# NUS-HPC-AI-Lab/VideoSys

Measured on AMD Instinct MI355X. Metric: videos/min (Open-Sora 512x512x64f, 30 denoise steps, DiT denoising only) + sec/denoise-step, higher is better.
Workload: dtype bf16; 1 GPU; open-sora-v1.2 STDiT3-XL/2 512x512x64f, latent [4,19,64,64], CFG batch 2 = 38912 token rows, 300 text tokens, depth 28; steps_per_video=30, parallelism=dsp1

## Files before the change

videosys_amd/csrc/rowwise.hip:

```cpp
#include "common.h"

#include <cstdlib>
#include "vsys_internal.h"

namespace vsys {
namespace {

template <int MAXV>
__global__ __launch_bounds__(256) void adaln_modulate_kernel(const bf16_t* __restrict__ x, const bf16_t* __restrict__ shift,
                                                             const bf16_t* __restrict__ scale, bf16_t* __restrict__ y,
                                                             int64_t rows, int C, int64_t rows_per_sample,
                                                             int64_t mod_stride, float eps) {
  const int lane = threadIdx.x & 63;
  const int64_t row = (int64_t)blockIdx.x * 4 + (threadIdx.x >> 6);
  if (row >= rows) return;
  const int nchunk = C >> 3;
  const bf16_t* xr = x + row * C;
  float v[MAXV][8];
  float s = 0.f;
#pragma unroll
  for (int i = 0; i < MAXV; ++i) {
    const int c = lane + 64 * i;
    if (c < nchunk) {
      uint4 u = *reinterpret_cast<const uint4*>(xr + c * 8);
// ... 184 lines not shown
    unpack8(*reinterpret_cast<const uint4*>(gate + b * gate_stride + alt + c * 8), g);
#pragma unroll
    for (int k = 0; k < 8; ++k) a[k] += bf2f(f2bf(g[k] * v[k]));
    reinterpret_cast<uint4*>(x)[i] = pack8(a);
  }
}

__global__ void im2col_patch_kernel(const float* __restrict__ z, int Bz, bf16_t* __restrict__ out, int B, int F, int Cin, int H,
                                    int W, int p) {
  const int Hp = H / p, Wp = W / p, K = Cin * p * p;
  const int64_t total = (int64_t)B * F * Hp * Wp * K;
  for (int64_t i = (int64_t)blockIdx.x * blockDim.x + threadIdx.x; i < total; i += (int64_t)gridDim.x * blockDim.x) {
    const int k = (int)(i % K);
    const int64_t tok = i / K;
    const int wp = (int)(tok % Wp), hp = (int)((tok / Wp) % Hp), f = (int)((tok / ((int64_t)Wp * Hp)) % F);
    const int b = (int)(tok / ((int64_t)Wp * Hp * F));
    const int dx = k % p, dy = (k / p) % p, c = k / (p * p);
    out[i] = f2bf(z[((((int64_t)(b % Bz) * F + f) * Cin + c) * H + hp * p + dy) * W + wp * p + dx]);
  }
}

__global__ void unpatchify_cvx_kernel(const bf16_t* __restrict__ x, int64_t ldx, float* __restrict__ out, int B, int F, int Hp,
                                      int Wp, int Cout, int p) {
  const int H = Hp * p, W = Wp * p;
  const int64_t total = (int64_t)B * F * Cout * H * W;
  for (int64_t i = (int64_t)blockIdx.x * blockDim.x + threadIdx.x; i < total; i += (int64_t)gridDim.x * blockDim.x) {
    const int w = (int)(i % W), h = (int)((i / W) % H), c = (int)((i / ((int64_t)W * H)) % Cout);
    const int64_t bf = i / ((int64_t)W * H * Cout);
    const int64_t tok = (bf * Hp + h / p) * Wp + w / p;
    out[i] = bf2f(x[tok * ldx + (c * p + h % p) * p + w % p]);
  }
}

__global__ void mod_table_kernel(const bf16_t* __restrict__ table, const bf16_t* __restrict__ t_mlp, bf16_t* __restrict__ out,
                                 int nblk, int B, int C6) {
  const int64_t i = (int64_t)blockIdx.x * blockDim.x + threadIdx.x;
  const int64_t total = (int64_t)nblk * B * C6;
  if (i >= total) return;
  const int c = (int)(i % C6);
  const int b = (int)((i / C6) % B);
  const int k = (int)(i / ((int64_t)C6 * B));
  out[i] = f2bf(bf2f(table[(int64_t)k * C6 + c]) + bf2f(t_mlp[(int64_t)b * C6 + c]));
}

__global__ void timestep_embedding_kernel(const float* __restrict__ t, bf16_t* __restrict__ out, int B, int dim) {
  const int i = blockIdx.x * blockDim.x + threadIdx.x;
  const int half = dim / 2;
  if (i >= B * half) return;
  const int b = i / half, k = i - b * half;
  const float f = expf(-9.210340371976184f * (float)k / (float)half);
  const float a = t[b] * f;
  out[(int64_t)b * dim + k] = f2bf(cosf(a));
  out[(int64_t)b * dim + half + k] = f2bf(sinf(a));
}

__global__ __launch_bounds__(256) void patch_embed_kernel(const float* __restrict__ x, int Bz, const bf16_t* __restrict__ w,
                                                          const bf16_t* __restrict__ bias, const bf16_t* __restrict__ pos,
                                                          bf16_t* __restrict__ out, int B, int Cin, int T, int H, int W,
                                                          int ph, int pw, int C, int s0, int Sl) {
  const int Hp = (H + ph - 1) / ph, Wp = (W + pw - 1) / pw;
  const int S = Hp * Wp;
  const int cchunks = C >> 3;
  const int64_t total = (int64_t)B * T * Sl * cchunks;
  const int64_t i = (int64_t)blockIdx.x * blockDim.x + threadIdx.x;
  if (i >= total) return;
  const int cc = (int)(i % cchunks);
  const int64_t tok = i / cchunks;
  const int s = s0 + (int)(tok % Sl);
  const int t = (int)((tok / Sl) % T);
  const int b = (int)(tok / ((int64_t)Sl * T));
  const int bz = b % Bz;
  if (s >= S) {
    *reinterpret_cast<uint4*>(out + tok * C + cc * 8) = make_uint4(0, 0, 0, 0);
    return;
  }
  const int hp = s / Wp, wp = s - hp * Wp;
  float acc[8];
  {
    float bb[8];
    unpack8(*reinterpret_cast<const uint4*>(bias + cc * 8), bb);
#pragma unroll
    for (int e = 0; e < 8; ++e) acc[e] = bb[e];
  }
  const int K = Cin * ph * pw;
  if (K == 16) {
    float xin[16];
#pragma unroll
    for (int k = 0; k < 16; ++k) {
      const int ci = k >> 2, dy = (k >> 1) & 1, dx = k & 1;
      const int hh = hp * 2 + dy, ww = wp * 2 + dx;
      xin[k] = 0.f;
      if (ph == 2 && pw == 2 && hh < H && ww < W) xin[k] = bf2f(f2bf(x[((((int64_t)bz * Cin + ci) * T + t) * H + hh) * W + ww]));
    }
    if (ph == 2 && pw == 2) {
#pragma unroll
      for (int e = 0; e < 8; ++e) {
        const bf16_t* wr = w + (int64_t)(cc * 8 + e) * 16;
        float wa[8], wb[8];
        unpack8(*reinterpret_cast<const uint4*>(wr), wa);
        unpack8(*reinterpret_cast<const uint4*>(wr + 8), wb);
#pragma unroll
        for (int k = 0; k < 8; ++k) acc[e] += xin[k] * wa[k] + xin[k + 8] * wb[k];
      }
    }
  }
  if (!(K == 16 && ph == 2 && pw == 2)) {
    for (int ci = 0; ci < Cin; ++ci)
      for (int dy = 0; dy < ph; ++dy)
        for (int dx = 0; dx < pw; ++dx) {
          const int hh = hp * ph + dy, ww = wp * pw + dx;
          float xv = 0.f;
          if (hh < H && ww < W) xv = bf2f(f2bf(x[((((int64_t)bz * Cin + ci) * T + t) * H + hh) * W + ww]));
          const int k = (ci * ph + dy) * pw + dx;
#pragma unroll
          for (int e = 0; e < 8; ++e) acc[e] += xv * bf2f(w[(int64_t)(cc * 8 + e) * K + k]);
        }
  }
  float pp[8];
  unpack8(*reinterpret_cast<const uint4*>(pos + (int64_t)s * C + cc * 8), pp);
#pragma unroll
  for (int e = 0; e < 8; ++e) acc[e] = bf2f(f2bf(acc[e])) + pp[e];
  *reinterpret_cast<uint4*>(out + tok * C + cc * 8) = pack8(acc);
}

template <int MAXV>
__global__ __launch_bounds__(256) void final_layer_kernel(const bf16_t* __restrict__ x, const bf16_t* __restrict__ table,
                                                          const bf16_t* __restrict__ tvec, const bf16_t* __restrict__ w,
                                                          const bf16_t* __restrict__ bias, float* __restrict__ out,
                                                          int B, int T, int Hp, int Wp, int H, int W, int ph, int pw,
                                                          int Cout, int C, float eps, int Sl, float* __restrict__ tokens) {
  const int lane = threadIdx.x & 63;
  const int S = Sl;
  const int64_t rows = (int64_t)B * T * S;
  const int64_t row = (int64_t)blockIdx.x * 4 + (threadIdx.x >> 6);
  if (row >= rows) return;
  const int nchunk = C >> 3;
  const bf16_t* xr = x + row * C;
  float v[MAXV][8];
  float s = 0.f;
#pragma unroll
  for (int i = 0; i < MAXV; ++i) {
    const int c = lane + 64 * i;
    if (c < nchunk) {
      unpack8(*reinterpret_cast<const uint4*>(xr + c * 8), v[i]);
#pragma unroll
      for (int e = 0; e < 8; ++e) s += v[i][e];
    } else {
#pragma unroll
      for (int e = 0; e < 8; ++e) v[i][e] = 0.f;
    }
  }
  const float mean = wave_sum(s) / (float)C;
  float q = 0.f;
#pragma unroll
  for (int i = 0; i < MAXV; ++i) {
    const int c = lane + 64 * i;
    if (c < nchunk) {
#pragma unroll
      for (int e = 0; e < 8; ++e) {
        float d = v[i][e] - mean;
        q += d * d;
      }
    }
  }
  const float rstd = rsqrtf(wave_sum(q) / (float)C + eps);
  const int b = (int)(row / ((int64_t)T * S));
#pragma unroll
  for (int i = 0; i < MAXV; ++i) {
    const int c = lane + 64 * i;
    if (c < nchunk) {
      float sh[8], sc[8], tt[8];
      unpack8(*reinterpret_cast<const uint4*>(table + c * 8), sh);
      unpack8(*reinterpret_cast<const uint4*>(table + C + c * 8), sc);
      unpack8(*reinterpret_cast<const uint4*>(tvec + (int64_t)b * C + c * 8), tt);
#pragma unroll
      for (int e = 0; e < 8; ++e) {
        const float shift = bf2f(f2bf(sh[e] + tt[e])), scale = bf2f(f2bf(sc[e] + tt[e]));
        v[i][e] = bf2f(f2bf((v[i][e] - mean) * rstd * (1.0f + scale) + shift));
      }
    }
  }
  const int NOUT = ph * pw * Cout;
  const int64_t tok = row % ((int64_t)T * S);
  const int t = (int)(tok / S), sidx = (int)(tok % S);
  const int hp = sidx / Wp, wp = sidx - hp * Wp;
  for (int n = 0; n < NOUT; ++n) {
    const bf16_t* wr = w + (int64_t)n * C;
    float d = 0.f;
#pragma unroll
    for (int i = 0; i < MAXV; ++i) {
      const int c = lane + 64 * i;
      if (c < nchunk) {
        float ww[8];
        unpack8(*reinterpret_cast<const uint4*>(wr + c * 8), ww);
#pragma unroll
        for (int e = 0; e < 8; ++e) d += v[i][e] * ww[e];
      }
    }
    d = wave_sum(d);
    if (lane == 0) {
      d = bf2f(f2bf(d + bf2f(bias[n])));
      if (tokens != nullptr) {
        tokens[row * NOUT + n] = d;
        continue;
      }
      const int co = n % Cout;
      const int dx = (n / Cout) % pw, dy = n / (Cout * pw);
      const int hh = hp * ph + dy, ww2 = wp * pw + dx;
      if (hh < H && ww2 < W) out[((((int64_t)b * Cout + co) * T + t) * H + hh) * W + ww2] = d;
    }
  }
}

__global__ void unpatchify_tokens_kernel(const float* __restrict__ tok, float* __restrict__ out, int P, int B, int T, int Sl,
                                         int Hp, int Wp, int H, int W, int ph, int pw, int Cout) {
  const int NOUT = ph * pw * Cout;
  const int64_t total = (int64_t)B * Cout * T * H * W;
  const int64_t i = (int64_t)blockIdx.x * blockDim.x + threadIdx.x;
  if (i >= total) return;
  const int ww = (int)(i % W), hh = (int)((i / W) % H), t = (int)((i / ((int64_t)W * H)) % T);
  const int co = (int)((i / ((int64_t)W * H * T)) % Cout), b = (int)(i / ((int64_t)W * H * T * Cout));
  const int hp = hh / ph, dy = hh - hp * ph, wp = ww / pw, dx = ww - wp * pw;
  const int s = hp * Wp + wp;
  const int r = s / Sl, j = s - r * Sl;
  const int n = (dy * pw + dx) * Cout + co;
  out[i] = tok[((((int64_t)r * B + b) * T + t) * Sl + j) * NOUT + n];
}

__global__ void cfg_euler_kernel(float* __restrict__ z, const float* __restrict__ model_out, int Bz, int Cin, int Cout,
                                 int64_t thw, float guidance, float dt) {
  const int64_t i = (int64_t)blockIdx.x * blockDim.x + threadIdx.x;
  const int64_t total = (int64_t)Bz * Cin * thw;
  if (i >= total) return;
  const int64_t sp = i % thw;
  const int c = (int)((i / thw) % Cin);
  const int b = (int)(i / (thw * Cin));
  const float cond = model_out[((int64_t)b * Cout + c) * thw + sp];
  const float unc = model_out[((int64_t)(b + Bz) * Cout + c) * thw + sp];
  z[i] = z[i] + (unc + guidance * (cond - unc)) * dt;
}

__global__ void cfg_axpby_kernel(float* __restrict__ z, const float* __restrict__ model_out, int Bz, int Cin, int Cout,
                                 int64_t thw, float guidance, float c_z, float c_eps, int cond_first) {
  const int64_t i = (int64_t)blockIdx.x * blockDim.x + threadIdx.x;
  const int64_t total = (int64_t)Bz * Cin * thw;
  if (i >= total) return;
  const int64_t sp = i % thw;
  const int c = (int)((i / thw) % Cin);
  const int b = (int)(i / (thw * Cin));
  const float h0 = model_out[((int64_t)b * Cout + c) * thw + sp];
  const float h1 = model_out[((int64_t)(b + Bz) * Cout + c) * thw + sp];
  const float cond = cond_first ? h0 : h1, unc = cond_first ? h1 : h0;
  z[i] = c_z * z[i] + c_eps * (unc + guidance * (cond - unc));
}

__global__ void add_bcast_rows_kernel(bf16_t* __restrict__ x, const bf16_t* __restrict__ e, int64_t rows, int C8, int64_t group,
                                      int64_t period) {
  const int64_t total = rows * C8;
  for (int64_t i = (int64_t)blockIdx.x * blockDim.x + threadIdx.x; i < total; i += (int64_t)gridDim.x * blockDim.x) {
    const int64_t r = i / C8;
    const int c = (int)(i - r * C8);
    const int64_t er = (r / group) % period;
    float a[8], b[8];
    unpack8(reinterpret_cast<const uint4*>(x)[i], a);
// ... 21 lines not shown
  for (int64_t i = (int64_t)blockIdx.x * blockDim.x + threadIdx.x; i < total; i += (int64_t)gridDim.x * blockDim.x) {
    const int64_t r = i / C8;
    const int c = (int)(i - r * C8) * 8;
    float x[8], y[8];
    unpack8(*reinterpret_cast<const uint4*>(a + r * lda + c), x);
    unpack8(*reinterpret_cast<const uint4*>(b + r * ldb + c), y);
#pragma unroll
    for (int e = 0; e < 8; ++e) x[e] = bf2f(f2bf(x[e] * scale)) + y[e];
    *reinterpret_cast<uint4*>(out + r * ldo + c) = pack8(x);
  }
}

__global__ void copy_4d_kernel(const bf16_t* __restrict__ src, bf16_t* __restrict__ dst, int n0, int n1, int n2, int C,
                               int64_t ss0, int64_t ss1, int64_t ss2, int64_t ds0, int64_t ds1, int64_t ds2,
                               int n1_valid, int n2_valid) {
  const int cch = C >> 3;
  const int64_t total = (int64_t)n0 * n1 * n2 * cch;
  for (int64_t i = (int64_t)blockIdx.x * blockDim.x + threadIdx.x; i < total; i += (int64_t)gridDim.x * blockDim.x) {
    const int c = (int)(i % cch);
    int64_t r = i / cch;
    const int i2 = (int)(r % n2);
    r /= n2;
    const int i1 = (int)(r % n1);
    const int i0 = (int)(r / n1);
    uint4 v = make_uint4(0, 0, 0, 0);
    if (i1 < n1_valid && i2 < n2_valid) v = *reinterpret_cast<const uint4*>(src + i0 * ss0 + i1 * ss1 + i2 * ss2 + c * 8);
    *reinterpret_cast<uint4*>(dst + i0 * ds0 + i1 * ds1 + i2 * ds2 + c * 8) = v;
  }
}

struct CopyBatch {
  int nops;
  CopyDesc d[VSYS_COPY_BATCH_MAX];
};
__global__ void copy_4d_batch_kernel(const bf16_t* __restrict__ src, bf16_t* __restrict__ dst, CopyBatch b) {
  const CopyDesc& o = b.d[blockIdx.y];
  const int cch = o.C >> 3;
  const int64_t total = (int64_t)o.n0 * o.n1 * o.n2 * cch;
  const bf16_t* s = src + o.src_off;
  bf16_t* d = dst + o.dst_off;
  for (int64_t i = (int64_t)blockIdx.x * blockDim.x + threadIdx.x; i < total; i += (int64_t)gridDim.x * blockDim.x) {
    const int c = (int)(i % cch);
    int64_t r = i / cch;
    const int i2 = (int)(r % o.n2);
    r /= o.n2;
    const int i1 = (int)(r % o.n1);
    const int i0 = (int)(r / o.n1);
    uint4 v = make_uint4(0, 0, 0, 0);
    if (i1 < o.n1_valid && i2 < o.n2_valid) v = *reinterpret_cast<const uint4*>(s + i0 * o.ss0 + i1 * o.ss1 + i2 * o.ss2 + c * 8);
    *reinterpret_cast<uint4*>(d + i0 * o.ds0 + i1 * o.ds1 + i2 * o.ds2 + c * 8) = v;
  }
}

}

int launch_copy_4d_batch(const bf16_t* src, bf16_t* dst, const CopyDesc* ops, int nops, hipStream_t stream) {
  if (nops <= 0) return 0;
  if (nops > VSYS_COPY_BATCH_MAX) return VSYS_ERR_SHAPE;
  CopyBatch b;
  b.nops = nops;
  int64_t most = 0;
  for (int i = 0; i < nops; ++i) {
    if (ops[i].C % 8 || ops[i].n0 < 0 || ops[i].n1 < 0 || ops[i].n2 < 0) return VSYS_ERR_SHAPE;
    b.d[i] = ops[i];
    const int64_t t = (int64_t)ops[i].n0 * ops[i].n1 * ops[i].n2 * (ops[i].C / 8);
    most = t > most ? t : most;
  }
  if (most <= 0) return 0;
  int64_t grid = (most + 255) / 256;
  if (grid > 2048) grid = 2048;
  hipLaunchKernelGGL(copy_4d_batch_kernel, dim3((unsigned)grid, (unsigned)nops), dim3(256), 0, stream, src, dst, b);
  return hipGetLastError() == hipSuccess ? 0 : VSYS_ERR_LAUNCH;
}

int launch_adaln_modulate(const bf16_t* x, const bf16_t* shift, const bf16_t* scale, bf16_t* y, int64_t rows, int C,
                          int64_t rows_per_sample, int64_t mod_stride, float eps, hipStream_t stream) {
  if (rows <= 0) return 0;
  if (C % 8 != 0 || C > 64 * 8 * 4 || rows_per_sample <= 0 || (mod_stride % 8)) return VSYS_ERR_SHAPE;
  if (C > 64 * 8 * 2 && C <= 64 * 8 * 3 && rows_per_sample % 2 == 0) {
    hipLaunchKernelGGL(adaln_modulate_rows_kernel<2>, dim3((unsigned)((rows + 7) / 8)), dim3(256), 0, stream, x, shift, scale, y, rows, C,
                       rows_per_sample, mod_stride, eps);
    return hipGetLastError() == hipSuccess ? 0 : VSYS_ERR_LAUNCH;
  }
  const unsigned grid = (unsigned)((rows + 3) / 4);
  if (C <= 64 * 8 * 2)
    hipLaunchKernelGGL(adaln_modulate_kernel<2>, dim3(grid), dim3(256), 0, stream, x, shift, scale, y, rows, C,
                       rows_per_sample, mod_stride, eps);
  else if (C <= 64 * 8 * 3)
    hipLaunchKernelGGL(adaln_modulate_kernel<3>, dim3(grid), dim3(256), 0, stream, x, shift, scale, y, rows, C,
                       rows_per_sample, mod_stride, eps);
  else
    hipLaunchKernelGGL(adaln_modulate_kernel<4>, dim3(grid), dim3(256), 0, stream, x, shift, scale, y, rows, C,
                       rows_per_sample, mod_stride, eps);
  return hipGetLastError() == hipSuccess ? 0 : VSYS_ERR_LAUNCH;
}

int launch_ln_modulate(const bf16_t* x, const bf16_t* ln_w, const bf16_t* ln_b, const bf16_t* shift, const bf16_t* scale,
                       bf16_t* y, int64_t rows, int C, int64_t rows_per_sample, int64_t mod_stride, int64_t seg_split,
                       int64_t mod_alt, float eps, hipStream_t stream) {
  if (rows <= 0) return 0;
  if (C % 8 != 0 || C > 64 * 8 * 6 || rows_per_sample <= 0 || (mod_stride % 8) || (mod_alt % 8)) return VSYS_ERR_SHAPE;
  if ((ln_w == nullptr) != (ln_b == nullptr) || (shift == nullptr) != (scale == nullptr)) return VSYS_ERR_ARG;
  const unsigned grid = (unsigned)((rows + 3) / 4);
#define VSYS_LNMOD(V)                                                                                                      \
  hipLaunchKernelGGL(ln_modulate_kernel<V>, dim3(grid), dim3(256), 0, stream, x, ln_w, ln_b, shift, scale, y, rows, C,       \
                     rows_per_sample, mod_stride, seg_split, mod_alt, eps)
// ... 10 lines not shown
  if (rows <= 0) return 0;
  if (C % 8 || rows_per_sample <= 0 || (gate_stride % 8) || (gate_alt % 8)) return VSYS_ERR_SHAPE;
  int64_t grid = (rows * (C / 8) + 255) / 256;
  if (grid > 2048 * 4) grid = 2048 * 4;
  hipLaunchKernelGGL(gate_add_rows_kernel, dim3((unsigned)grid), dim3(256), 0, stream, x, y, gate, rows, C / 8, rows_per_sample,
                     gate_stride, seg_split, gate_alt);
  return hipGetLastError() == hipSuccess ? 0 : VSYS_ERR_LAUNCH;
}

int launch_im2col_patch(const float* z, int Bz, bf16_t* out, int B, int F, int Cin, int H, int W, int p, hipStream_t stream) {
  if (p <= 0 || H % p || W % p || Bz <= 0) return VSYS_ERR_SHAPE;
  const int64_t total = (int64_t)B * F * (H / p) * (W / p) * Cin * p * p;
  if (total <= 0) return 0;
  int64_t grid = (total + 255) / 256;
  if (grid > 2048 * 8) grid = 2048 * 8;
  hipLaunchKernelGGL(im2col_patch_kernel, dim3((unsigned)grid), dim3(256), 0, stream, z, Bz, out, B, F, Cin, H, W, p);
  return hipGetLastError() == hipSuccess ? 0 : VSYS_ERR_LAUNCH;
}

int launch_unpatchify_cvx(const bf16_t* x, int64_t ldx, float* out, int B, int F, int Hp, int Wp, int Cout, int p,
                          hipStream_t stream) {
  const int64_t total = (int64_t)B * F * Cout * Hp * p * Wp * p;
  if (total <= 0) return 0;
  int64_t grid = (total + 255) / 256;
  if (grid > 2048 * 8) grid = 2048 * 8;
  hipLaunchKernelGGL(unpatchify_cvx_kernel, dim3((unsigned)grid), dim3(256), 0, stream, x, ldx, out, B, F, Hp, Wp, Cout, p);
  return hipGetLastError() == hipSuccess ? 0 : VSYS_ERR_LAUNCH;
}

int launch_mod_table(const bf16_t* table, const bf16_t* t_mlp, bf16_t* out, int nblk, int B, int C6, hipStream_t stream) {
  const int64_t total = (int64_t)nblk * B * C6;
  if (total <= 0) return 0;
  hipLaunchKernelGGL(mod_table_kernel, dim3((unsigned)((total + 255) / 256)), dim3(256), 0, stream, table, t_mlp, out, nblk,
                     B, C6);
  return hipGetLastError() == hipSuccess ? 0 : VSYS_ERR_LAUNCH;
}

int launch_timestep_embedding(const float* t, bf16_t* out, int B, int dim, hipStream_t stream) {
  if (dim % 2) return VSYS_ERR_SHAPE;
  const int total = B * (dim / 2);
  if (total <= 0) return 0;
  hipLaunchKernelGGL(timestep_embedding_kernel, dim3((total + 127) / 128), dim3(128), 0, stream, t, out, B, dim);
  return hipGetLastError() == hipSuccess ? 0 : VSYS_ERR_LAUNCH;
}

int launch_patch_embed(const float* x, int Bz, const bf16_t* w, const bf16_t* bias, const bf16_t* pos, bf16_t* out, int B,
                       int Cin, int T, int H, int W, int ph, int pw, int C, int s0, int Sl, hipStream_t stream) {
  if (C % 8 || Bz <= 0 || s0 < 0) return VSYS_ERR_SHAPE;
  const int Hp = (H + ph - 1) / ph, Wp = (W + pw - 1) / pw;
  if (Sl < 0) Sl = Hp * Wp;
  const int64_t total = (int64_t)B * T * Sl * (C / 8);
  if (total <= 0) return 0;
  if ((total + 255) / 256 > 0x7fffffff) return VSYS_ERR_SHAPE;
  hipLaunchKernelGGL(patch_embed_kernel, dim3((unsigned)((total + 255) / 256)), dim3(256), 0, stream, x, Bz, w, bias, pos, out,
                     B, Cin, T, H, W, ph, pw, C, s0, Sl);
  return hipGetLastError() == hipSuccess ? 0 : VSYS_ERR_LAUNCH;
}

int launch_unpatchify_tokens(const float* tok, float* out, int P, int B, int T, int Sl, int Hp, int Wp, int H, int W, int ph,
                             int pw, int Cout, hipStream_t stream) {
  if (P <= 0 || Sl <= 0 || (int64_t)P * Sl < (int64_t)Hp * Wp) return VSYS_ERR_SHAPE;
  const int64_t total = (int64_t)B * Cout * T * H * W;
  if (total <= 0) return 0;
  if ((total + 255) / 256 > 0x7fffffff) return VSYS_ERR_SHAPE;
  hipLaunchKernelGGL(unpatchify_tokens_kernel, dim3((unsigned)((total + 255) / 256)), dim3(256), 0, stream, tok, out, P, B, T, Sl,
                     Hp, Wp, H, W, ph, pw, Cout);
  return hipGetLastError() == hipSuccess ? 0 : VSYS_ERR_LAUNCH;
}

int launch_final_layer(const bf16_t* x, const bf16_t* table, const bf16_t* tvec, const bf16_t* w, const bf16_t* bias,
                       float* out, int B, int T, int Hp, int Wp, int H, int W, int ph, int pw, int Cout, int C, float eps,
                       int Sl, float* tokens, hipStream_t stream) {
  if (C % 8 != 0 || C > 64 * 8 * 4) return VSYS_ERR_SHAPE;
  if (Sl < 0) Sl = Hp * Wp;
  if (tokens == nullptr && Sl != Hp * Wp) return VSYS_ERR_ARG;
  const int64_t rows = (int64_t)B * T * Sl;
  if (rows <= 0) return 0;
  const unsigned grid = (unsigned)((rows + 3) / 4);
  if (C <= 64 * 8 * 2)
    hipLaunchKernelGGL(final_layer_kernel<2>, dim3(grid), dim3(256), 0, stream, x, table, tvec, w, bias, out, B, T, Hp, Wp,
                       H, W, ph, pw, Cout, C, eps, Sl, tokens);
  else if (C <= 64 * 8 * 3)
    hipLaunchKernelGGL(final_layer_kernel<3>, dim3(grid), dim3(256), 0, stream, x, table, tvec, w, bias, out, B, T, Hp, Wp,
                       H, W, ph, pw, Cout, C, eps, Sl, tokens);
  else
    hipLaunchKernelGGL(final_layer_kernel<4>, dim3(grid), dim3(256), 0, stream, x, table, tvec, w, bias, out, B, T, Hp, Wp,
                       H, W, ph, pw, Cout, C, eps, Sl, tokens);
  return hipGetLastError() == hipSuccess ? 0 : VSYS_ERR_LAUNCH;
}

int launch_cfg_euler(float* z, const float* model_out, int Bz, int Cin, int Cout, int64_t thw, float guidance, float dt,
                     hipStream_t stream) {
  const int64_t total = (int64_t)Bz * Cin * thw;
  if (total <= 0) return 0;
  hipLaunchKernelGGL(cfg_euler_kernel, dim3((unsigned)((total + 255) / 256)), dim3(256), 0, stream, z, model_out, Bz, Cin,
                     Cout, thw, guidance, dt);
  return hipGetLastError() == hipSuccess ? 0 : VSYS_ERR_LAUNCH;
}

int launch_cfg_axpby(float* z, const float* model_out, int Bz, int Cin, int Cout, int64_t thw, float guidance, float c_z,
                     float c_eps, int cond_first, hipStream_t stream) {
  const int64_t total = (int64_t)Bz * Cin * thw;
  if (total <= 0) return 0;
  hipLaunchKernelGGL(cfg_axpby_kernel, dim3((unsigned)((total + 255) / 256)), dim3(256), 0, stream, z, model_out, Bz, Cin,
                     Cout, thw, guidance, c_z, c_eps, cond_first);
  return hipGetLastError() == hipSuccess ? 0 : VSYS_ERR_LAUNCH;
}

int launch_add_bcast_rows(bf16_t* x, const bf16_t* e, int64_t rows, int C, int64_t group, int64_t period, hipStream_t stream) {
  if (rows <= 0) return 0;
  if (C % 8 || group <= 0 || period <= 0) return VSYS_ERR_SHAPE;
  int64_t grid = (rows * (C / 8) + 255) / 256;
  if (grid > 2048 * 4) grid = 2048 * 4;
  hipLaunchKernelGGL(add_bcast_rows_kernel, dim3((unsigned)grid), dim3(256), 0, stream, x, e, rows, C / 8, group, period);
  return hipGetLastError() == hipSuccess ? 0 : VSYS_ERR_LAUNCH;
}

int launch_add_rows(bf16_t* x, const bf16_t* y, int64_t n, hipStream_t stream) {
  if (n <= 0) return 0;
  if (n % 8) return VSYS_ERR_SHAPE;
  const int64_t n8 = n / 8;
  int64_t grid = (n8 + 255) / 256;
  if (grid > 2048 * 4) grid = 2048 * 4;
  hipLaunchKernelGGL(add_rows_kernel, dim3((unsigned)grid), dim3(256), 0, stream, x, y, n8);
  return hipGetLastError() == hipSuccess ? 0 : VSYS_ERR_LAUNCH;
}

int launch_scale_add_rows(const bf16_t* a, int64_t lda, const bf16_t* b, int64_t ldb, bf16_t* out, int64_t ldo, int64_t rows, int C,
                          float scale, hipStream_t stream) {
  if (rows < 0 || C < 0) return VSYS_ERR_SHAPE;
// ... 25 lines not shown
```

Baseline: 21.73 videos/min.

## Add LDS-staged final layer and register-tiled patch-embed kernels

Adds a specialized patch-embed kernel for 4-channel 2x2 patches. It keeps each thread's weight slice in registers, stages input patches in shared memory, prefetches positional embeddings, and writes the result once per CFG batch copy. Adds a final-layer kernel that stages the projection weights and modulation vectors in LDS, prefetches the next row, and reduces 16 outputs at once with butterfly shuffles instead of one wave reduction per output. Both kernels size their grids from the CU count and are selected by default unless an environment flag requests the reference path. These are small per-step kernels compared with the 28 transformer blocks, so their share of end-to-end time is limited.

```diff
diff --git a/videosys_amd/csrc/rowwise.hip b/videosys_amd/csrc/rowwise.hip
--- a/videosys_amd/csrc/rowwise.hip
+++ b/videosys_amd/csrc/rowwise.hip
@@ -418,6 +418,258 @@
       if (hh < H && ww2 < W) out[((((int64_t)b * Cout + co) * T + t) * H + hh) * W + ww2] = d;
     }
   }
+}
+
+
+constexpr int PE_TOKENS = 64;
+constexpr int PE_THREADS = 512;
+__global__ __launch_bounds__(PE_THREADS, 2) void patch_embed_k16_kernel(
+    const float* __restrict__ x, int Bz, const bf16_t* __restrict__ w, const bf16_t* __restrict__ bias,
+    const bf16_t* __restrict__ pos, bf16_t* __restrict__ out, int B, int T, int H, int W, int C, int s0, int Sl, int cpb, int tpb,
+    int ntok, int U) {
+  __shared__ __attribute__((aligned(16))) float xs[PE_TOKENS * 16];
+  constexpr int Cin = 4;
+  const int Hp = (H + 1) / 2, Wp = (W + 1) / 2;
+  const int S = Hp * Wp;
+  const int cchunks = C >> 3;
+  const int u0 = blockIdx.x * ntok;
+  const int u1 = U - u0 < ntok ? U : u0 + ntok;
+  const int slot = threadIdx.x / cpb;
+  const int cc = blockIdx.y * cpb + (threadIdx.x - slot * cpb);
+  const bool active = slot < tpb && cc < cchunks;
+  float wf[8][16], bb[8];
+  int j = 0, t = 0, bz = 0;
+  int ucur = u0 + slot;
+  uint4 upn = make_uint4(0, 0, 0, 0);
+  if (active) {
+#pragma unroll
+    for (int e = 0; e < 8; ++e) {
+      const bf16_t* wr = w + (int64_t)(cc * 8 + e) * 16;
+      unpack8(*reinterpret_cast<const uint4*>(wr), wf[e]);
+      unpack8(*reinterpret_cast<const uint4*>(wr + 8), wf[e] + 8);
+    }
+    unpack8(*reinterpret_cast<const uint4*>(bias + cc * 8), bb);
+    j = ucur % Sl;
+    t = (ucur / Sl) % T;
+    bz = ucur / Sl / T;
+    if (ucur < u1 && s0 + j < S) upn = *reinterpret_cast<const uint4*>(pos + (int64_t)(s0 + j) * C + cc * 8);
+  }
+  const int batch = PE_TOKENS / tpb * tpb;
+  for (int ub = u0; ub < u1; ub += batch) {
+    const int n = u1 - ub < batch ? u1 - ub : batch;
+    for (int idx = threadIdx.x; idx < n * 16; idx += blockDim.x) {
+      const int k = idx & 15;
+      const int u = ub + (idx >> 4);
+      const int s = s0 + u % Sl;
+      const int tt = (u / Sl) % T;
+      const int bb0 = u / Sl / T;
+      float xv = 0.f;
+      if (s < S) {
+        const int hp = s / Wp, wp = s - hp * Wp;
+        const int ci = k >> 2, dy = (k >> 1) & 1, dx = k & 1;
+        const int hh = hp * 2 + dy, ww = wp * 2 + dx;
+        if (hh < H && ww < W) xv = bf2f(f2bf(x[((((int64_t)bb0 * Cin + ci) * T + tt) * H + hh) * W + ww]));
+      }
+      xs[idx] = xv;
+    }
+    __syncthreads();
+    if (active) {
+      for (; ucur < ub + n; ucur += tpb) {
+        const int i = ucur - ub;
+        const int s = s0 + j;
+        const uint4 up = upn;
+        int jn = j + tpb, tn = t, bn = bz;
+        while (jn >= Sl) {
+          jn -= Sl;
+          if (++tn == T) {
+            tn = 0;
+            ++bn;
+          }
+        }
+        if (u1 - ucur > tpb && s0 + jn < S) upn = *reinterpret_cast<const uint4*>(pos + (int64_t)(s0 + jn) * C + cc * 8);
+        uint4 o = make_uint4(0, 0, 0, 0);
+        if (s < S) {
+          float xin[16];
+#pragma unroll
+          for (int q = 0; q < 4; ++q) {
+            const float4 f = *reinterpret_cast<const float4*>(xs + i * 16 + q * 4);
+            xin[q * 4 + 0] = f.x; xin[q * 4 + 1] = f.y; xin[q * 4 + 2] = f.z; xin[q * 4 + 3] = f.w;
+          }
+          float acc[8];
+#pragma unroll
+          for (int e = 0; e < 8; ++e) acc[e] = bb[e];
+#pragma unroll
+          for (int e = 0; e < 8; ++e) {
+            const float* wa = wf[e];
+            const float* wb = wf[e] + 8;
+#pragma unroll
+            for (int k = 0; k < 8; ++k) acc[e] += xin[k] * wa[k] + xin[k + 8] * wb[k];
+          }
+          float pp[8];
+          unpack8(up, pp);
+#pragma unroll
+          for (int e = 0; e < 8; ++e) acc[e] = bf2f(f2bf(acc[e])) + pp[e];
+          o = pack8(acc);
+        }
+        for (int b = bz; b < B; b += Bz) *reinterpret_cast<uint4*>(out + (((int64_t)b * T + t) * Sl + j) * C + cc * 8) = o;
+        j = jn;
+        t = tn;
+        bz = bn;
+      }
+    }
+    __syncthreads();
+  }
+}
+
+constexpr int FL_THREADS = 512;
+__device__ __forceinline__ void fmac(float& d, float a, float b) { asm("v_fmac_f32_e32 %0, %1, %2" : "+v"(d) : "v"(a), "v"(b)); }
+constexpr int FL_LOG2G = 4, FL_G = 1 << FL_LOG2G;
+template <int MAXV>
+__global__ __launch_bounds__(FL_THREADS, 4) void final_layer_lds_kernel(
+    const bf16_t* __restrict__ x, const bf16_t* __restrict__ table, const bf16_t* __restrict__ tvec, const bf16_t* __restrict__ w,
+    const bf16_t* __restrict__ bias, float* __restrict__ out, int B, int T, int Hp, int Wp, int H, int W, int ph, int pw, int Cout,
+    int C, float eps, int Sl, float* __restrict__ tokens, int rpw, int gps) {
+  extern __shared__ __attribute__((aligned(16))) uint4 fl_lds[];
+  const int lane = threadIdx.x & 63, wave = threadIdx.x >> 6;
+  const int S = Sl;
+  const int nchunk = C >> 3;
+  const int NOUT = ph * pw * Cout;
+  const int b = blockIdx.x / gps;
+  const int g = blockIdx.x - b * gps;
+  const int64_t TS = (int64_t)T * S;
+  const int NP = (NOUT + FL_G - 1) / FL_G * FL_G;
+  for (int idx = threadIdx.x; idx < NP * nchunk; idx += FL_THREADS) {
+    const int nn = idx / nchunk, c = idx - nn * nchunk;
+    fl_lds[c * (NP + 1) + nn] = nn < NOUT ? reinterpret_cast<const uint4*>(w)[idx] : make_uint4(0, 0, 0, 0);
+  }
+  uint4* mod = fl_lds + nchunk * (NP + 1);
+  for (int c = threadIdx.x; c < nchunk; c += FL_THREADS) {
+    float sh[8], sc[8], tt[8];
+    unpack8(*reinterpret_cast<const uint4*>(table + c * 8), sh);
+    unpack8(*reinterpret_cast<const uint4*>(table + C + c * 8), sc);
+    unpack8(*reinterpret_cast<const uint4*>(tvec + (int64_t)b * C + c * 8), tt);
+#pragma unroll
+    for (int e = 0; e < 8; ++e) {
+      sh[e] = sh[e] + tt[e];
+      sc[e] = sc[e] + tt[e];
+    }
+    mod[c] = pack8(sh);
+    mod[nchunk + c] = pack8(sc);
+  }
+  __syncthreads();
+  const int64_t tok_end = (int64_t)(g + 1) * rpw < TS ? (int64_t)(g + 1) * rpw : TS;
+  int64_t tok = (int64_t)g * rpw + wave;
+  if (tok >= tok_end) return;
+  uint4 un[MAXV];
+#pragma unroll
+  for (int i = 0; i < MAXV; ++i) {
+    const int c = lane + 64 * i;
+    un[i] = c < nchunk ? *reinterpret_cast<const uint4*>(x + ((int64_t)b * TS + tok) * C + c * 8) : make_uint4(0, 0, 0, 0);
+  }
+  for (; tok < tok_end; tok += FL_THREADS / 64) {
+    const int64_t row = (int64_t)b * TS + tok;
+    float v[MAXV][8];
+    float s = 0.f;
+#pragma unroll
+    for (int i = 0; i < MAXV; ++i) {
+      const int c = lane + 64 * i;
+      if (c < nchunk) {
+        unpack8(un[i], v[i]);
+#pragma unroll
+        for (int e = 0; e < 8; ++e) s += v[i][e];
+      } else {
+#pragma unroll
+        for (int e = 0; e < 8; ++e) v[i][e] = 0.f;
+      }
+    }
+    if (tok + FL_THREADS / 64 < tok_end) {
+#pragma unroll
+      for (int i = 0; i < MAXV; ++i) {
+        const int c = lane + 64 * i;
+        if (c < nchunk) un[i] = *reinterpret_cast<const uint4*>(x + (row + FL_THREADS / 64) * C + c * 8);
+      }
+    }
+    const float mean = wave_sum(s) / (float)C;
+    float q = 0.f;
+#pragma unroll
+    for (int i = 0; i < MAXV; ++i) {
+      const int c = lane + 64 * i;
+      if (c < nchunk) {
+#pragma unroll
+        for (int e = 0; e < 8; ++e) {
+          float d = v[i][e] - mean;
+          q += d * d;
+        }
+      }
+    }
+    const float rstd = rsqrtf(wave_sum(q) / (float)C + eps);
+#pragma unroll
+    for (int i = 0; i < MAXV; ++i) {
+      const int c = lane + 64 * i;
+      if (c < nchunk) {
+        float sh[8], sc[8];
+        unpack8(mod[c], sh);
+        unpack8(mod[nchunk + c], sc);
+#pragma unroll
+        for (int e = 0; e < 8; ++e) {
+          const float shift = sh[e], scale = sc[e];
+          v[i][e] = bf2f(f2bf((v[i][e] - mean) * rstd * (1.0f + scale) + shift));
+        }
+      }
+    }
+    const int t = (int)(tok / S), sidx = (int)(tok % S);
+    const int hp = sidx / Wp, wp = sidx - hp * Wp;
+    for (int n0 = 0; n0 < NOUT; n0 += FL_G) {
+      float d[FL_G];
+#pragma unroll
+      for (int j = 0; j < FL_G; ++j) d[j] = 0.f;
+#pragma unroll
+      for (int i = 0; i < MAXV; ++i) {
+        const int c = lane + 64 * i;
+        if (c < nchunk) {
+#pragma unroll
+          for (int j = 0; j < FL_G; ++j) {
+            float ww[8];
+            unpack8(fl_lds[c * (NP + 1) + n0 + j], ww);
+#pragma unroll
+            for (int e = 0; e < 8; ++e) fmac(d[j], v[i][e], ww[e]);
+          }
+        }
+      }
+#pragma unroll
+      for (int st = 0; st < FL_LOG2G; ++st) {
+        const int h = (FL_G / 2) >> st, o = 32 >> st;
+        const bool up = (lane & o) != 0;
+#pragma unroll
+        for (int j = 0; j < h; ++j) {
+          const float lo = d[j], hi = d[j + h];
+          const float keep = up ? hi : lo;
+          const float send = up ? lo : hi;
+          d[j] = keep + __shfl_xor(send, o, 64);
+        }
+      }
+      float r = d[0];
+#pragma unroll
+      for (int o = 32 >> FL_LOG2G; o > 0; o >>= 1) r += __shfl_xor(r, o, 64);
+      const int n = n0 + (lane >> (6 - FL_LOG2G));
+      if ((lane & ((64 >> FL_LOG2G) - 1)) == 0 && n < NOUT) {
+        r = bf2f(f2bf(r + bf2f(bias[n])));
+        if (tokens != nullptr) {
+          tokens[row * NOUT + n] = r;
+        } else {
+          const int co = n % Cout;
+          const int dx = (n / Cout) % pw, dy = n / (Cout * pw);
+          const int hh = hp * ph + dy, ww2 = wp * pw + dx;
+          if (hh < H && ww2 < W) out[((((int64_t)b * Cout + co) * T + t) * H + hh) * W + ww2] = r;
+        }
+      }
+    }
+  }
+}
+
+inline bool rowwise_ref_route() {
+  static const bool ref = [] { const char* e = getenv("VSYS_ROWWISE_REF"); return e && e[0] == '1'; }();
+  return ref;
 }
 
 __global__ void unpatchify_tokens_kernel(const float* __restrict__ tok, float* __restrict__ out, int P, int B, int T, int Sl,
@@ -661,6 +913,29 @@
   const int64_t total = (int64_t)B * T * Sl * (C / 8);
   if (total <= 0) return 0;
   if ((total + 255) / 256 > 0x7fffffff) return VSYS_ERR_SHAPE;
+  if (Cin == 4 && ph == 2 && pw == 2 && !rowwise_ref_route()) {
+    const int cchunks = C / 8;
+    const int cpb = cchunks < PE_THREADS ? cchunks : PE_THREADS;
+    int tpb = 1, threads = (cpb + 63) / 64 * 64;
+    for (int k = 2; k * cpb <= PE_THREADS; ++k) {
+      const int th = (k * cpb + 63) / 64 * 64;
+      if ((int64_t)k * threads > (int64_t)tpb * th) {
+        tpb = k;
+        threads = th;
+      }
+    }
+    if (tpb > PE_TOKENS) tpb = PE_TOKENS;
+    const int64_t U = (int64_t)(Bz < B ? Bz : B) * T * Sl;
+    if (U + PE_THREADS > 0x7fffffff) return VSYS_ERR_SHAPE;
+    const int gy = (cchunks + cpb - 1) / cpb;
+    const int64_t want = cu_count_this_device() / gy > 0 ? cu_count_this_device() / gy : 1;
+    int64_t ntok = (U + want - 1) / want;
+    if (ntok < tpb) ntok = tpb;
+    const int64_t gx = (U + ntok - 1) / ntok;
+    hipLaunchKernelGGL(patch_embed_k16_kernel, dim3((unsigned)gx, (unsigned)gy), dim3(threads), 0, stream, x, Bz, w, bias, pos, out, B,
+                       T, H, W, C, s0, Sl, cpb, tpb, (int)ntok, (int)U);
+    return hipGetLastError() == hipSuccess ? 0 : VSYS_ERR_LAUNCH;
+  }
   hipLaunchKernelGGL(patch_embed_kernel, dim3((unsigned)((total + 255) / 256)), dim3(256), 0, stream, x, Bz, w, bias, pos, out,
                      B, Cin, T, H, W, ph, pw, C, s0, Sl);
   return hipGetLastError() == hipSuccess ? 0 : VSYS_ERR_LAUNCH;
@@ -685,6 +960,31 @@
   if (tokens == nullptr && Sl != Hp * Wp) return VSYS_ERR_ARG;
   const int64_t rows = (int64_t)B * T * Sl;
   if (rows <= 0) return 0;
+  const int64_t nout = (int64_t)ph * pw * Cout;
+  const int64_t lds = ((nout + FL_G - 1) / FL_G * FL_G + 1) * (C / 8) * 16 + 2 * C * 2;
+  if (nout > 0 && lds <= 160 * 1024 && !rowwise_ref_route()) {
+    static std::atomic<unsigned long long> attr_seen{0};
+    for (DeviceOnce once(attr_seen); once.todo(); once.done()) {
+      (void)hipFuncSetAttribute((const void*)final_layer_lds_kernel<2>, hipFuncAttributeMaxDynamicSharedMemorySize, 160 * 1024);
+      (void)hipFuncSetAttribute((const void*)final_layer_lds_kernel<3>, hipFuncAttributeMaxDynamicSharedMemorySize, 160 * 1024);
+      (void)hipFuncSetAttribute((const void*)final_layer_lds_kernel<4>, hipFuncAttributeMaxDynamicSharedMemorySize, 160 * 1024);
+    }
+    const int64_t TS = (int64_t)T * Sl;
+    int64_t gps = (2 * cu_count_this_device() + B - 1) / B;
+    int64_t rpw = (TS + gps - 1) / gps;
+    if (rpw < FL_THREADS / 64) rpw = FL_THREADS / 64;
+    gps = (TS + rpw - 1) / rpw;
+    if (gps * B > 0x7fffffff || rpw > 0x7fffffff) return VSYS_ERR_SHAPE;
+    const dim3 fgrid((unsigned)(gps * B));
+#define VSYS_FINAL(V)                                                                                                       \
+  hipLaunchKernelGGL(final_layer_lds_kernel<V>, fgrid, dim3(FL_THREADS), (size_t)lds, stream, x, table, tvec, w, bias, out, B, T, \
+                     Hp, Wp, H, W, ph, pw, Cout, C, eps, Sl, tokens, (int)rpw, (int)gps)
+    if (C <= 64 * 8 * 2) VSYS_FINAL(2);
+    else if (C <= 64 * 8 * 3) VSYS_FINAL(3);
+    else VSYS_FINAL(4);
+#undef VSYS_FINAL
+    return hipGetLastError() == hipSuccess ? 0 : VSYS_ERR_LAUNCH;
+  }
   const unsigned grid = (unsigned)((rows + 3) / 4);
   if (C <= 64 * 8 * 2)
     hipLaunchKernelGGL(final_layer_kernel<2>, dim3(grid), dim3(256), 0, stream, x, table, tvec, w, bias, out, B, T, Hp, Wp,
```

Result: no change. 21.90 videos/min, median of 6 (+0.8%).

## Add persistent patch-embed and final-layer kernels with register/LDS weight reuse

Applied to the files above, without the earlier changes.

Adds a persistent patch-embed kernel for 2x2x4 patches that keeps each thread's weights in registers and double-buffers input pixels through shared memory. It also adds a final-layer kernel for 32 outputs that caches the projection weights in LDS (optionally as fp32), processes two rows per wave with packed f32x2 math, and reduces the results with a shuffle butterfly. Both are meant to cut repeated weight loads and per-row launch overhead at the model's two ends. They run by default unless an environment flag selects the old path. The FP contraction order is pinned so results match the reference rounding, and the kernels add LDS and register pressure.

```diff
diff --git a/videosys_amd/csrc/rowwise.hip b/videosys_amd/csrc/rowwise.hip
--- a/videosys_amd/csrc/rowwise.hip
+++ b/videosys_amd/csrc/rowwise.hip
@@ -260,6 +260,20 @@
   const float a = t[b] * f;
   out[(int64_t)b * dim + k] = f2bf(cosf(a));
   out[(int64_t)b * dim + half + k] = f2bf(sinf(a));
+}
+
+__device__ __forceinline__ void patch16_channels8(float* acc, const float* x, const float (*w)[16]) {
+#pragma clang fp contract(off)
+#pragma unroll
+  for (int e = 0; e < 8; ++e) {
+    const bool lo_rounded = e < 6 && (e & 1) == 0;
+#pragma unroll
+    for (int k = 0; k < 8; ++k) {
+      const float u = lo_rounded ? __builtin_fmaf(x[k + 8], w[e][k + 8], x[k] * w[e][k])
+                                 : __builtin_fmaf(x[k], w[e][k], x[k + 8] * w[e][k + 8]);
+      acc[e] = acc[e] + u;
+    }
+  }
 }
 
 __global__ __launch_bounds__(256) void patch_embed_kernel(const float* __restrict__ x, int Bz, const bf16_t* __restrict__ w,
@@ -301,15 +315,14 @@
       if (ph == 2 && pw == 2 && hh < H && ww < W) xin[k] = bf2f(f2bf(x[((((int64_t)bz * Cin + ci) * T + t) * H + hh) * W + ww]));
     }
     if (ph == 2 && pw == 2) {
+      float wf[8][16];
 #pragma unroll
       for (int e = 0; e < 8; ++e) {
         const bf16_t* wr = w + (int64_t)(cc * 8 + e) * 16;
-        float wa[8], wb[8];
-        unpack8(*reinterpret_cast<const uint4*>(wr), wa);
-        unpack8(*reinterpret_cast<const uint4*>(wr + 8), wb);
-#pragma unroll
-        for (int k = 0; k < 8; ++k) acc[e] += xin[k] * wa[k] + xin[k + 8] * wb[k];
-      }
+        unpack8(*reinterpret_cast<const uint4*>(wr), wf[e]);
+        unpack8(*reinterpret_cast<const uint4*>(wr + 8), wf[e] + 8);
+      }
+      patch16_channels8(acc, xin, wf);
     }
   }
   if (!(K == 16 && ph == 2 && pw == 2)) {
@@ -329,6 +342,121 @@
 #pragma unroll
   for (int e = 0; e < 8; ++e) acc[e] = bf2f(f2bf(acc[e])) + pp[e];
   *reinterpret_cast<uint4*>(out + tok * C + cc * 8) = pack8(acc);
+}
+
+constexpr int PE16_THREADS = 512, PE16_MAXTOK = 16;
+__global__ __launch_bounds__(PE16_THREADS) void patch_embed16_kernel(const float* __restrict__ x, int Bz, const bf16_t* __restrict__ w,
+                                                                     const bf16_t* __restrict__ bias, const bf16_t* __restrict__ pos,
+                                                                     bf16_t* __restrict__ out, int T, int H, int W, int C, int s0,
+                                                                     int Sl, int ntok, int toks, int passes, int passes_per_wg) {
+  __shared__ float xs[2][2 * PE16_MAXTOK * 16];
+  const int tid = threadIdx.x;
+  const int cchunks = C >> 3;
+  const int Hp = (H + 1) >> 1, Wp = (W + 1) >> 1;
+  const int S = Hp * Wp;
+  const int slot = tid / cchunks, cc = tid - slot * cchunks;
+  const bool active = slot < toks;
+  float wf[8][16], bb[8];
+  if (active) {
+#pragma unroll
+    for (int e = 0; e < 8; ++e) {
+      const bf16_t* wr = w + (int64_t)(cc * 8 + e) * 16;
+      unpack8(*reinterpret_cast<const uint4*>(wr), wf[e]);
+      unpack8(*reinterpret_cast<const uint4*>(wr + 8), wf[e] + 8);
+    }
+    unpack8(*reinterpret_cast<const uint4*>(bias + cc * 8), bb);
+  } else {
+#pragma unroll
+    for (int e = 0; e < 8; ++e) {
+      bb[e] = 0.f;
+#pragma unroll
+      for (int k = 0; k < 16; ++k) wf[e][k] = 0.f;
+    }
+  }
+  const int p_begin = blockIdx.x * passes_per_wg;
+  const int p_end = p_begin + passes_per_wg < passes ? p_begin + passes_per_wg : passes;
+  const int lw = tid >> 4, lk = tid & 15;
+  const bool loader = lw < 2 * toks;
+  auto fetch = [&](int p) -> float {
+    const int tok = p * 2 * toks + lw;
+    if (!loader || tok >= ntok) return 0.f;
+    const int bt = tok / Sl;
+    const int s = s0 + (tok - bt * Sl);
+    if (s >= S) return 0.f;
+    const int b = bt / T, t = bt - b * T;
+    const int bz = b % Bz;
+    const int hp = s / Wp, wp = s - hp * Wp;
+    const int ci = lk >> 2, dy = (lk >> 1) & 1, dx = lk & 1;
+    const int hh = hp * 2 + dy, ww = wp * 2 + dx;
+    if (hh < H && ww < W) return x[((((int64_t)bz * 4 + ci) * T + t) * H + hh) * W + ww];
+    return 0.f;
+  };
+  if (p_begin >= p_end) return;
+  const int step_mod = (2 * toks) % Sl;
+  int rem[2] = {(p_begin * 2 * toks + slot) % Sl, (p_begin * 2 * toks + toks + slot) % Sl};
+  auto fetch_pos = [&](int p, int* s_out, uint4* pp) {
+#pragma unroll
+    for (int u = 0; u < 2; ++u) {
+      const int tok = p * 2 * toks + u * toks + slot;
+      s_out[u] = -1;
+      pp[u] = make_uint4(0, 0, 0, 0);
+      if (active && tok < ntok) {
+        const int s = s0 + rem[u];
+        s_out[u] = s < S ? s : S;
+        if (s < S) pp[u] = *reinterpret_cast<const uint4*>(pos + (int64_t)s * C + cc * 8);
+      }
+      rem[u] += step_mod;
+      rem[u] -= rem[u] >= Sl ? Sl : 0;
+    }
+  };
+  float xn = fetch(p_begin);
+  int sn[2];
+  uint4 pn[2];
+  fetch_pos(p_begin, sn, pn);
+  uint4 od[2] = {make_uint4(0, 0, 0, 0), make_uint4(0, 0, 0, 0)};
+  bool have[2] = {false, false};
+  int buf = 0;
+  for (int p = p_begin; p <= p_end; ++p) {
+    int sc[2] = {-1, -1};
+    uint4 pc[2] = {pn[0], pn[1]};
+    if (p < p_end) {
+      if (loader) xs[buf][tid] = bf2f(f2bf(xn));
+      __syncthreads();
+      sc[0] = sn[0];
+      sc[1] = sn[1];
+      if (p + 1 < p_end) {
+        xn = fetch(p + 1);
+        fetch_pos(p + 1, sn, pn);
+      }
+    }
+#pragma unroll
+    for (int u = 0; u < 2; ++u) {
+      if (have[u]) *reinterpret_cast<uint4*>(out + ((int64_t)(p - 1) * 2 * toks + u * toks + slot) * C + cc * 8) = od[u];
+      have[u] = sc[u] >= 0;
+    }
+    if (p == p_end) break;
+#pragma unroll
+    for (int u = 0; u < 2; ++u) {
+      od[u] = make_uint4(0, 0, 0, 0);
+      if (sc[u] >= 0 && sc[u] < S) {
+        float xin[16], acc[8], pp[8];
+        const float4* xr = reinterpret_cast<const float4*>(&xs[buf][(u * toks + slot) * 16]);
+#pragma unroll
+        for (int j = 0; j < 4; ++j) {
+          const float4 q = xr[j];
+          xin[4 * j] = q.x; xin[4 * j + 1] = q.y; xin[4 * j + 2] = q.z; xin[4 * j + 3] = q.w;
+        }
+#pragma unroll
+        for (int e = 0; e < 8; ++e) acc[e] = bb[e];
+        patch16_channels8(acc, xin, wf);
+        unpack8(pc[u], pp);
+#pragma unroll
+        for (int e = 0; e < 8; ++e) acc[e] = bf2f(f2bf(acc[e])) + pp[e];
+        od[u] = pack8(acc);
+      }
+    }
+    buf ^= 1;
+  }
 }
 
 template <int MAXV>
@@ -416,6 +544,209 @@
       const int dx = (n / Cout) % pw, dy = n / (Cout * pw);
       const int hh = hp * ph + dy, ww2 = wp * pw + dx;
       if (hh < H && ww2 < W) out[((((int64_t)b * Cout + co) * T + t) * H + hh) * W + ww2] = d;
+    }
+  }
+}
+
+template <int MAXV>
+__device__ __forceinline__ void final32_norm_row(const uint4* u, float (*v)[8], int lane, int nchunk, int C, float eps,
+                                                 const uint4* shp, const uint4* scp) {
+#pragma clang fp contract(off)
+  float s = 0.f;
+#pragma unroll
+  for (int i = 0; i < MAXV; ++i) {
+    unpack8(u[i], v[i]);
+    if (lane + 64 * i < nchunk) {
+#pragma unroll
+      for (int e = 0; e < 8; ++e) s += v[i][e];
+    }
+  }
+  const float mean = wave_sum(s) / (float)C;
+  float q = 0.f;
+#pragma unroll
+  for (int i = 0; i < MAXV; ++i) {
+    if (lane + 64 * i < nchunk) {
+#pragma unroll
+      for (int e = 0; e < 8; ++e) {
+        const float d = v[i][e] - mean;
+        const float dd = d * d;
+        q = q + dd;
+      }
+    }
+  }
+  const float rstd = rsqrtf(wave_sum(q) / (float)C + eps);
+#pragma unroll
+  for (int i = 0; i < MAXV; ++i) {
+    if (lane + 64 * i < nchunk) {
+      float shift[8], scale[8];
+      unpack8(shp[i], shift);
+      unpack8(scp[i], scale);
+#pragma unroll
+      for (int e = 0; e < 8; ++e) {
+        const float nrm = (v[i][e] - mean) * rstd;
+        v[i][e] = bf2f(f2bf(__builtin_fmaf(nrm, 1.0f + scale[e], shift[e])));
+      }
+    }
+  }
+}
+
+template <int MAXV>
+__device__ __forceinline__ void final32_sample(const bf16_t* __restrict__ table, const bf16_t* __restrict__ tvec, int b, int C,
+                                               int lane, int nchunk, uint4* shp, uint4* scp) {
+#pragma unroll
+  for (int i = 0; i < MAXV; ++i) {
+    const int c = lane + 64 * i;
+    if (c < nchunk) {
+      float sh[8], sc[8], tt[8];
+      unpack8(*reinterpret_cast<const uint4*>(table + c * 8), sh);
+      unpack8(*reinterpret_cast<const uint4*>(table + C + c * 8), sc);
+      unpack8(*reinterpret_cast<const uint4*>(tvec + (int64_t)b * C + c * 8), tt);
+#pragma unroll
+      for (int e = 0; e < 8; ++e) {
+        sh[e] += tt[e];
+        sc[e] += tt[e];
+      }
+      shp[i] = pack8(sh);
+      scp[i] = pack8(sc);
+    }
+  }
+}
+
+template <int MAXV, bool WF32>
+__global__ __launch_bounds__(WF32 ? 512 : 256) void final_layer32_kernel(const bf16_t* __restrict__ x, const bf16_t* __restrict__ table,
+                                                            const bf16_t* __restrict__ tvec, const bf16_t* __restrict__ w,
+                                                            const bf16_t* __restrict__ bias, float* __restrict__ out, int T,
+                                                            int Wp, int H, int W, int ph, int pw, int Cout, int C, float eps,
+                                                            int Sl, float* __restrict__ tokens, int rows, int pairs_per_wg) {
+#pragma clang fp contract(off)
+  extern __shared__ uint4 wl[];
+  constexpr int NT = WF32 ? 512 : 256;
+  const int lane = threadIdx.x & 63;
+  const int wave = __builtin_amdgcn_readfirstlane(threadIdx.x >> 6);
+  const int nchunk = C >> 3;
+  for (int j = threadIdx.x; j < 32 * nchunk; j += NT) {
+    const uint4 g = reinterpret_cast<const uint4*>(w)[j];
+    if (WF32) {
+      float f[8];
+      unpack8(g, f);
+      const int nn = j / nchunk, c = j - nn * nchunk;
+      reinterpret_cast<float4*>(wl)[(2 * nn) * nchunk + c] = make_float4(f[0], f[1], f[2], f[3]);
+      reinterpret_cast<float4*>(wl)[(2 * nn + 1) * nchunk + c] = make_float4(f[4], f[5], f[6], f[7]);
+    } else {
+      wl[j] = g;
+    }
+  }
+  __syncthreads();
+  const int npairs = (rows + 1) >> 1;
+  const int pair_begin = blockIdx.x * pairs_per_wg;
+  const int pair_end = pair_begin + pairs_per_wg < npairs ? pair_begin + pairs_per_wg : npairs;
+  const int TS = T * Sl;
+  const int n = lane & 31, half = lane >> 5;
+  const float bn = bf2f(bias[n]);
+  const int co = n % Cout, dx = (n / Cout) % pw, dy = n / (Cout * pw);
+
+  uint4 shp[MAXV], scp[MAXV];
+#pragma unroll
+  for (int i = 0; i < MAXV; ++i) shp[i] = scp[i] = make_uint4(0, 0, 0, 0);
+  int bcur = -1;
+  auto load_rows = [&](int pair, uint4 (*u)[MAXV]) {
+#pragma unroll
+    for (int r = 0; r < 2; ++r) {
+      int row = 2 * pair + r;
+      row = row < rows ? row : rows - 1;
+#pragma unroll
+      for (int i = 0; i < MAXV; ++i) {
+        const int c = lane + 64 * i;
+        u[r][i] = c < nchunk ? *reinterpret_cast<const uint4*>(x + (int64_t)row * C + c * 8) : make_uint4(0, 0, 0, 0);
+      }
+    }
+  };
+
+  int pair = pair_begin + wave;
+  if (pair >= pair_end) return;
+  constexpr bool PF = !(WF32 && MAXV >= 3);
+  uint4 un[2][MAXV];
+  if (PF) load_rows(pair, un);
+  constexpr int NW = NT / 64;
+  for (; pair < pair_end; pair += NW) {
+    uint4 uc[2][MAXV];
+    if (PF) {
+#pragma unroll
+      for (int r = 0; r < 2; ++r)
+#pragma unroll
+        for (int i = 0; i < MAXV; ++i) uc[r][i] = un[r][i];
+      if (pair + NW < pair_end) load_rows(pair + NW, un);
+    } else {
+      load_rows(pair, uc);
+    }
+    const int row0 = 2 * pair;
+    const int row1 = row0 + 1 < rows ? row0 + 1 : row0;
+    const int b0 = row0 / TS, b1 = row1 / TS;
+    float va[MAXV][8], vb[MAXV][8];
+    if (b0 != bcur) final32_sample<MAXV>(table, tvec, b0, C, lane, nchunk, shp, scp);
+    final32_norm_row<MAXV>(uc[0], va, lane, nchunk, C, eps, shp, scp);
+    if (b1 != b0) final32_sample<MAXV>(table, tvec, b1, C, lane, nchunk, shp, scp);
+    final32_norm_row<MAXV>(uc[1], vb, lane, nchunk, C, eps, shp, scp);
+    bcur = b1;
+    f32x2 v2[MAXV][8];
+#pragma unroll
+    for (int i = 0; i < MAXV; ++i)
+#pragma unroll
+      for (int e = 0; e < 8; ++e) {
+        v2[i][e] = f32x2{va[i][e], vb[i][e]};
+        asm volatile("" : "+v"(v2[i][e]));
+      }
+
+    float a[64];
+#pragma unroll
+    for (int nn = 0; nn < 32; ++nn) {
+      f32x2 d = {0.f, 0.f};
+#pragma unroll
+      for (int i = 0; i < MAXV; ++i) {
+        const int c = lane + 64 * i;
+        if (c < nchunk) {
+          float ww[8];
+          if (WF32) {
+            const float4 lo = reinterpret_cast<const float4*>(wl)[(2 * nn) * nchunk + c];
+            const float4 hi = reinterpret_cast<const float4*>(wl)[(2 * nn + 1) * nchunk + c];
+            ww[0] = lo.x; ww[1] = lo.y; ww[2] = lo.z; ww[3] = lo.w;
+            ww[4] = hi.x; ww[5] = hi.y; ww[6] = hi.z; ww[7] = hi.w;
+          } else {
+            unpack8(wl[nn * nchunk + c], ww);
+          }
+#pragma unroll
+          for (int e = 0; e < 8; ++e) {
+            const f32x2 prod = v2[i][e] * f32x2{ww[e], ww[e]};
+            d = d + prod;
+          }
+        }
+      }
+      a[nn] = d.x;
+      a[32 + nn] = d.y;
+    }
+#pragma unroll
+    for (int o = 32; o > 0; o >>= 1) {
+      const bool up = (lane & o) != 0;
+#pragma unroll
+      for (int j = 0; j < o; ++j) {
+        const float keep = up ? a[j + o] : a[j];
+        const float send = up ? a[j] : a[j + o];
+        a[j] = keep + __shfl_xor(send, o, 64);
+      }
+    }
+    const int row = row0 + half;
+    if (row < rows) {
+      const float d = bf2f(f2bf(a[0] + bn));
+      if (tokens != nullptr) {
+        tokens[(int64_t)row * 32 + n] = d;
+      } else {
+        const int b = half ? b1 : b0;
+        const int tok = row - b * TS;
+        const int t = tok / Sl, sidx = tok - t * Sl;
+        const int hp = sidx / Wp, wp = sidx - hp * Wp;
+        const int hh = hp * ph + dy, ww2 = wp * pw + dx;
+        if (hh < H && ww2 < W) out[((((int64_t)b * Cout + co) * T + t) * H + hh) * W + ww2] = d;
+      }
     }
   }
 }
@@ -545,6 +876,14 @@
   }
 }
 
+#ifndef VSYS_FINAL32_F32_IMAGE
+#define VSYS_FINAL32_F32_IMAGE 1
+#endif
+bool rowwise_v1() {
+  static const bool on = [] { const char* e = getenv("VSYS_ROWWISE_V1"); return e && e[0] == '1'; }();
+  return on;
+}
+
 }
 
 int launch_copy_4d_batch(const bf16_t* src, bf16_t* dst, const CopyDesc* ops, int nops, hipStream_t stream) {
@@ -661,6 +1000,18 @@
   const int64_t total = (int64_t)B * T * Sl * (C / 8);
   if (total <= 0) return 0;
   if ((total + 255) / 256 > 0x7fffffff) return VSYS_ERR_SHAPE;
+  const int64_t ntok = (int64_t)B * T * Sl;
+  if (!rowwise_v1() && Cin == 4 && ph == 2 && pw == 2 && C / 8 <= PE16_THREADS && ntok <= (1 << 30)) {
+    int toks = PE16_THREADS / (C / 8);
+    toks = toks < PE16_MAXTOK ? toks : PE16_MAXTOK;
+    const int passes = (int)((ntok + 2 * toks - 1) / (2 * toks));
+    const int slots = cu_count_this_device();
+    const int per_wg = (passes + slots - 1) / slots;
+    const int grid = (passes + per_wg - 1) / per_wg;
+    hipLaunchKernelGGL(patch_embed16_kernel, dim3((unsigned)grid), dim3(PE16_THREADS), 0, stream, x, Bz, w, bias, pos, out, T, H, W, C,
+                       s0, Sl, (int)ntok, toks, passes, per_wg);
+    return hipGetLastError() == hipSuccess ? 0 : VSYS_ERR_LAUNCH;
+  }
   hipLaunchKernelGGL(patch_embed_kernel, dim3((unsigned)((total + 255) / 256)), dim3(256), 0, stream, x, Bz, w, bias, pos, out,
                      B, Cin, T, H, W, ph, pw, C, s0, Sl);
   return hipGetLastError() == hipSuccess ? 0 : VSYS_ERR_LAUNCH;
@@ -685,6 +1036,35 @@
   if (tokens == nullptr && Sl != Hp * Wp) return VSYS_ERR_ARG;
   const int64_t rows = (int64_t)B * T * Sl;
   if (rows <= 0) return 0;
+  if (!rowwise_v1() && ph * pw * Cout == 32 && rows <= (1 << 30)) {
+    const bool wf32 = VSYS_FINAL32_F32_IMAGE && 128 * C <= 144 * 1024;
+    const int lds = (wf32 ? 128 : 64) * C;
+    static std::atomic<unsigned long long> attr_seen{0};
+    for (DeviceOnce once(attr_seen); once.todo(); once.done()) {
+      (void)hipFuncSetAttribute((const void*)final_layer32_kernel<2, true>, hipFuncAttributeMaxDynamicSharedMemorySize, 144 * 1024);
+      (void)hipFuncSetAttribute((const void*)final_layer32_kernel<3, true>, hipFuncAttributeMaxDynamicSharedMemorySize, 144 * 1024);
+      (void)hipFuncSetAttribute((const void*)final_layer32_kernel<2, false>, hipFuncAttributeMaxDynamicSharedMemorySize, 64 * 1024);
+      (void)hipFuncSetAttribute((const void*)final_layer32_kernel<3, false>, hipFuncAttributeMaxDynamicSharedMemorySize, 64 * 1536);
+      (void)hipFuncSetAttribute((const void*)final_layer32_kernel<4, false>, hipFuncAttributeMaxDynamicSharedMemorySize, 64 * 2048);
+    }
+    const int nw = wf32 ? 8 : 4;
+    const int npairs = (int)((rows + 1) / 2);
+    const int groups = (npairs + nw - 1) / nw;
+    const int slots = (lds <= 80 * 1024 ? 2 : 1) * cu_count_this_device();
+    const int per_wg = nw * ((groups + slots - 1) / slots);
+    const int grid32 = (npairs + per_wg - 1) / per_wg;
+#define VSYS_FINAL32(V, F)                                                                                                          \
+  hipLaunchKernelGGL((final_layer32_kernel<V, F>), dim3((unsigned)grid32), dim3(F ? 512 : 256), lds, stream, x, table, tvec, w, bias, \
+                     out, T, Wp, H, W, ph, pw, Cout, C, eps, Sl, tokens, (int)rows, per_wg)
+    if (wf32) {
+      if (C <= 64 * 8 * 2) VSYS_FINAL32(2, true);
+      else VSYS_FINAL32(3, true);
+    } else if (C <= 64 * 8 * 2) VSYS_FINAL32(2, false);
+    else if (C <= 64 * 8 * 3) VSYS_FINAL32(3, false);
+    else VSYS_FINAL32(4, false);
+#undef VSYS_FINAL32
+    return hipGetLastError() == hipSuccess ? 0 : VSYS_ERR_LAUNCH;
+  }
   const unsigned grid = (unsigned)((rows + 3) / 4);
   if (C <= 64 * 8 * 2)
     hipLaunchKernelGGL(final_layer_kernel<2>, dim3(grid), dim3(256), 0, stream, x, table, tvec, w, bias, out, B, T, Hp, Wp,
```

Result: no change. 21.01 videos/min before, 21.16 videos/min after (median of 6 runs) (+0.7%).
